# lazear/sage

Hardware: AMD Instinct MI355X
Metric: spectra/sec (whole node), fragment-index search-and-score, human tryptic narrow search (higher is better)
Workload: dtype f32

## Files before the change

include/sage_hip.h:

```cpp
#ifndef SAGE_HIP_H
#define SAGE_HIP_H

#include <stddef.h>
#include <stdint.h>

#ifdef __cplusplus
extern "C" {
#endif

#define SAGE_HIP_ABI_VERSION 6

enum {
    SAGE_HIP_OK = 0,
    SAGE_HIP_ERR_INVALID = 1,
    SAGE_HIP_ERR_NO_DEVICE = 2,
    SAGE_HIP_ERR_HIP = 3,
    SAGE_HIP_ERR_UNSUPPORTED = 4,
    SAGE_HIP_ERR_OOM = 5,
    SAGE_HIP_ERR_INTERNAL = 6
};

enum { SAGE_TOL_PPM = 0, SAGE_TOL_PCT = 1, SAGE_TOL_DA = 2 };
typedef struct SageTolerance {
    int32_t kind;
// ... 173 lines not shown

typedef struct SageTiming {
    float prelim_ms;
    float rescore_ms;
    float total_ms;
    uint32_t n_launches;
    uint32_t n_wide;
    uint32_t arena_entries;
    uint32_t n_retry;
    float retry_ms;
    uint32_t n_tied;
    uint32_t n_ways;
} SageTiming;
int sage_hip_last_timing(const SageScorer* scorer, SageTiming* out);
int sage_hip_scorer_set_timing_interval(SageScorer* scorer, uint32_t every);

int sage_hip_host_alloc(uint64_t bytes, void** out);
void sage_hip_host_free(void* p);

int sage_hip_debug_phase_cycles(SageScorer* scorer, unsigned long long* out32);
int sage_hip_debug_prune_counters(SageScorer* scorer, unsigned long long* out4);
int sage_hip_debug_filter_counters(SageScorer* scorer, unsigned long long* out4);
int sage_hip_debug_heavy_counters(SageScorer* scorer, unsigned long long* out2);

typedef struct SageRescoreInput {
    uint64_t n;
    const SageFeature* features;
    const float* aligned_rt;
    const float* delta_rt_model;
    const float* delta_ims_model;
    SageTolerance precursor_tol;
    const uint32_t* peptide_key;
    uint32_t n_peptide_keys;
    const uint32_t* protein_key;
    uint32_t n_protein_keys;
} SageRescoreInput;

typedef struct SageRescoreOutput {
    float* discriminant_score;
    float* posterior_error;
    float* spectrum_q;
    float* peptide_q;
    float* protein_q;
    uint32_t* order;
    uint64_t passing_spectrum;
    uint64_t passing_peptide;
// ... 178 lines not shown
```

sage_amd/_lib.py:

```python
import ctypes as C
import os

import numpy as np

from . import build as _build

c_float_p = C.POINTER(C.c_float)
c_u8_p = C.POINTER(C.c_uint8)
c_u32_p = C.POINTER(C.c_uint32)
c_u64_p = C.POINTER(C.c_uint64)


class SageTolerance(C.Structure):
    _fields_ = [("kind", C.c_int32), ("lo", C.c_float), ("hi", C.c_float)]


class SageTheoretical(C.Structure):
    _fields_ = [("peptide_index", C.c_uint32), ("fragment_mz", C.c_float)]


class SageDbParams(C.Structure):
    _fields_ = [
        ("bucket_size", C.c_uint64),
        ("missed_cleavages", C.c_int32),
# ... 254 lines not shown
        "sage_hip_scorer_create": (C.c_int, [vp, C.POINTER(SageScorerParams), C.POINTER(vp)]),
        "sage_hip_scorer_destroy": (None, [vp]),
        "sage_hip_scorer_clone": (C.c_int, [vp, C.POINTER(vp)]),
        "sage_hip_score_batch": (C.c_int, [vp, C.POINTER(SageSpectrumBatch), vp, c_u32_p]),
        "sage_hip_batch_upload": (C.c_int, [vp, C.POINTER(SageSpectrumBatch), C.POINTER(vp)]),
        "sage_hip_batch_free": (None, [vp]),
        "sage_hip_batch_process_upload": (C.c_int, [vp, C.POINTER(SageRawBatch), C.c_uint64, C.c_int, C.c_float, C.c_uint32,
                                                    C.POINTER(vp), c_u32_p]),
        "sage_hip_batch_download": (C.c_int, [vp, c_u64_p, c_float_p, c_float_p, c_float_p]),
        "sage_hip_batch_upload_kinds": (C.c_int, [vp, C.POINTER(SageSpectrumBatch), c_u8_p, C.POINTER(vp)]),
        "sage_hip_batch_process_upload_kinds": (C.c_int, [vp, C.POINTER(SageRawBatch), c_u8_p, C.c_uint64, C.c_int, C.c_float,
                                                          C.c_uint32, C.POINTER(vp), c_u32_p]),
        "sage_hip_score_batch_kinds": (C.c_int, [vp, C.POINTER(SageSpectrumBatch), c_u8_p, vp, c_u32_p]),
        "sage_hip_score_resident": (C.c_int, [vp, vp, vp, c_u32_p]),
        "sage_hip_initial_hits": (C.c_int, [vp, vp, c_u64_p, C.c_uint32, c_u32_p, c_u64_p, c_u64_p]),
        "sage_hip_last_timing": (C.c_int, [vp, C.POINTER(SageTiming)]),
        "sage_hip_scorer_set_timing_interval": (C.c_int, [vp, C.c_uint32]),
        "sage_hip_annotate_resident": (C.c_int, [vp, vp, vp, c_u32_p, C.POINTER(SageFragments)]),
        "sage_hip_quick_score_resident": (C.c_int, [vp, vp, C.c_int, c_u8_p]),
        "sage_hip_debug_phase_cycles": (C.c_int, [vp, c_u64_p]),
        "sage_hip_debug_prune_counters": (C.c_int, [vp, c_u64_p]),
        "sage_hip_debug_filter_counters": (C.c_int, [vp, c_u64_p]),
        "sage_hip_debug_heavy_counters": (C.c_int, [vp, c_u64_p]),
        "sage_hip_host_alloc": (C.c_int, [C.c_uint64, C.POINTER(vp)]),
        "sage_hip_host_free": (None, [vp]),
        "sage_hip_rescore": (C.c_int, [C.c_int, C.POINTER(SageRescoreInput), C.POINTER(SageRescoreOutput)]),
        "sage_hip_hostdb_competition_keys": (C.c_int, [vp, c_u32_p, C.c_uint64, c_u32_p, c_u32_p, c_u32_p, c_u32_p]),
        "sage_hip_predict_rt": (C.c_int, [C.c_int, C.POINTER(SageRtInput), C.POINTER(SageRtOutput)]),
        "sage_hip_hostdb_feature_peptides": (C.c_int, [vp, c_u32_p, C.c_uint64, c_u64_p, c_u8_p, c_float_p]),
        "sage_hip_mzml_read": (C.c_int, [C.c_char_p, C.c_uint32, C.c_int, C.POINTER(vp)]),
        "sage_hip_mzml_view": (C.c_int, [vp, C.POINTER(SageRawBatch)]),
        "sage_hip_mzml_check_searchable": (C.c_int, [vp]),
        "sage_hip_mzml_spectrum_id": (C.c_char_p, [vp, C.c_uint64]),
        "sage_hip_mzml_free": (None, [vp]),
        "sage_hip_mzml_read_sn": (C.c_int, [C.c_char_p, C.c_uint32, C.c_int, C.c_int, C.POINTER(vp)]),
        "sage_hip_mzml_ion_injection_time": (C.c_float, [vp, C.c_uint64]),
        "sage_hip_mzml_precursor_ref": (C.c_char_p, [vp, C.c_uint64]),
        "sage_hip_mgf_read": (C.c_int, [C.c_char_p, C.c_uint32, C.POINTER(vp)]),
        "sage_hip_mzml_isolation_kinds": (C.c_int, [vp, c_u8_p]),
        "sage_hip_mzml_charge_zero": (C.c_int, [vp, c_u8_p]),
        "sage_hip_parse_f32": (C.c_int, [C.c_char_p, C.c_uint64, c_float_p]),
        "sage_hip_tmt": (C.c_int, [C.c_int, C.POINTER(SageTmtInput), C.POINTER(SageTmtOutput)]),
        "sage_hip_write_tmt": (C.c_int, [C.c_char_p, C.POINTER(C.c_char_p), C.c_uint32, C.c_uint64, c_u32_p, C.POINTER(C.c_char_p),
                                         c_float_p, c_float_p, C.POINTER(C.c_char_p), C.c_uint32]),
        "sage_hip_write_results": (C.c_int, [C.c_char_p, C.c_int, vp, vp, C.c_uint64, c_u64_p, c_u64_p, C.POINTER(C.c_char_p),
                                             C.c_uint32, C.POINTER(C.c_char_p), C.POINTER(SagePostColumns)]),
# ... 3 lines not shown
        "sage_hip_mzml_has_mobility": (C.c_int, [vp, c_u8_p]),
        "sage_hip_write_lfq": (C.c_int, [C.c_char_p, vp, C.POINTER(SageLfqOutput), c_u64_p, C.c_uint64, C.POINTER(C.c_char_p),
                                         C.c_uint32]),
        "sage_hip_fasta_num_targets": (C.c_int, [C.c_char_p, C.POINTER(SageDbParams), c_u64_p]),
        "sage_hip_prefilter_chunk_size": (C.c_int, [C.c_char_p, C.POINTER(SageDbParams), C.c_uint64, c_u64_p]),
        "sage_hip_hostdb_build_chunk": (C.c_int, [C.c_char_p, C.POINTER(SageDbParams), C.c_uint64, C.c_uint64, C.POINTER(vp)]),
        "sage_hip_hostdb_merge_kept": (C.c_int, [C.POINTER(vp), C.POINTER(c_u8_p), C.c_uint32, C.POINTER(SageDbParams),
                                                 C.POINTER(vp)]),
    }
    for name, (res, args) in sig.items():
        fn = getattr(lib, name)
        fn.restype = res
        fn.argtypes = args
    _lib = lib
    return lib


EXPORTED_SYMBOLS = [
    "sage_hip_last_error", "sage_hip_abi_version", "sage_hip_hostdb_build", "sage_hip_hostdb_free",
    "sage_hip_hostdb_view", "sage_hip_hostdb_peptide_string", "sage_hip_hostdb_peptide_proteins",
    "sage_hip_hostdb_peptide_info", "sage_hip_process_ms2", "sage_hip_device_count", "sage_hip_db_create", "sage_hip_db_destroy",
    "sage_hip_db_device_bytes", "sage_hip_scorer_create", "sage_hip_scorer_destroy", "sage_hip_scorer_clone", "sage_hip_score_batch",
    "sage_hip_batch_upload", "sage_hip_batch_free", "sage_hip_batch_process_upload", "sage_hip_batch_download", "sage_hip_score_resident", "sage_hip_initial_hits",
    "sage_hip_last_timing", "sage_hip_scorer_set_timing_interval", "sage_hip_annotate_resident", "sage_hip_quick_score_resident", "sage_hip_debug_phase_cycles", "sage_hip_debug_prune_counters", "sage_hip_debug_filter_counters", "sage_hip_debug_heavy_counters", "sage_hip_host_alloc", "sage_hip_host_free",
    "sage_hip_rescore", "sage_hip_hostdb_competition_keys", "sage_hip_fasta_num_targets", "sage_hip_prefilter_chunk_size",
    "sage_hip_hostdb_build_chunk", "sage_hip_hostdb_merge_kept", "sage_hip_predict_rt", "sage_hip_hostdb_feature_peptides",
    "sage_hip_write_results", "sage_hip_mzml_read", "sage_hip_mzml_view", "sage_hip_mzml_check_searchable", "sage_hip_mzml_spectrum_id", "sage_hip_mzml_free",
    "sage_hip_lfq", "sage_hip_write_lfq", "sage_hip_mzml_read_sn", "sage_hip_mzml_ion_injection_time", "sage_hip_mzml_precursor_ref",
    "sage_hip_tmt", "sage_hip_write_tmt", "sage_hip_mgf_read", "sage_hip_mzml_isolation_kinds", "sage_hip_mzml_charge_zero",
    "sage_hip_parse_f32", "sage_hip_batch_upload_kinds", "sage_hip_batch_process_upload_kinds", "sage_hip_score_batch_kinds",
    "sage_hip_lfq_im", "sage_hip_mzml_mobility", "sage_hip_mzml_has_mobility",
]


def check(rc):
    if rc != 0:
        msg = load().sage_hip_last_error()
        raise SageHipError(f"libsage_hip status {rc}: {msg.decode() if msg else ''}")


def as_ptr(arr, ctype):
    return arr.ctypes.data_as(C.POINTER(ctype))
```

sage_amd/csrc/capi.hip:

```cpp
#include <hip/hip_runtime.h>
#include <algorithm>
#include <atomic>
#include <cmath>
#include <chrono>
#include <cstring>
#include <memory>
#include <future>
#include <mutex>
#include <string>
#include <vector>

#include "crlog.h"
#include "device_types.h"
#define HIP_FAILED(e, what) fail(status_of(e), std::string(what) + ": " + hipGetErrorString(e))
#include "hip_host.h"
#include "host_db.hpp"

using namespace sagehip;

namespace {

thread_local std::string g_last_error;

int fail(int code, const std::string& msg) {
// ... 53 lines not shown
    DevBuf<uint64_t> pm_off;
    std::vector<float> h_pep_mono;
    DevBuf<SageTheoretical> tm_frag;
    DevBuf<uint32_t> tm_lut;
    DevBuf<SageTheoretical> tm2_frag;
    DevBuf<sagecore::LutWord> tm2_l1;
    DevBuf<uint32_t> tm2_pos;
    uint32_t max_ions = 0;
    uint32_t max_len = 0;
    uint32_t ion_lo_bits = 0xFFFFFFFFu, ion_hi_bits = 0;
    DevDbView view{};
    uint64_t bytes = 0;
};

struct WorkSet {
    DevBuf<uint64_t> cand;
    DevBuf<uint32_t> cand_len, totals, status, queue, retry, item_of, ready;
    uint32_t epoch = 0;
    DevBuf<QueryRec> qrec;
    DevBuf<uint16_t> seeds;
    DevBuf<uint64_t> qres;
    DevBuf<uint32_t> arena;
    DevBuf<uint32_t> cnt_store;
    DevBuf<float> winbuf;
    DevBuf<unsigned char> hugebuf;
    uint32_t cap_tie = 0;
    uint32_t cap_n = 0;
    uint32_t cap_wide = 0;
};

struct OutSet {
    DevBuf<SageFeature> features;
    DevBuf<uint32_t> out_count;
    DevBuf<uint32_t> counters;
    uint32_t* h_counters = nullptr;
    uint32_t* h_counters_view = nullptr;
    bool counters_clean = false;
    Pinned h_out;
    Event ev[5];
    Event comp_done, down_done;
    bool in_flight = false, two_pass = false, with_rescore = false;
    bool fused = false;
    bool wide_launched = true;
    bool timed = true;
    bool retry_deferred = false;
    bool huge = false;
    uint32_t n = 0;
    ~OutSet() {
        if (h_counters) (void)hipHostFree(h_counters);
// ... 36 lines not shown
    bool retry_likely = true;
    uint32_t timing_every = 1;
    uint64_t timing_calls = 0;
    bool timed = true;
    float kept_prelim_ms = 0.f, kept_rescore_ms = 0.f, kept_retry_ms = 0.f;
    DevBuf<double> lnfact;
    DevBuf<unsigned long long> dbg;
    uint32_t tile_blocks = 0;
    uint32_t tile_blocks8 = 0;
    bool cnt8 = true;
    bool reuse_counts = true;
    SageTiming timing{};
    bool exact_always = false;
    bool one_launch = false;
    uint32_t kstride = 64;
    bool two_lanes = true;
    uint32_t search_lag = 0;
    bool sched_desc_forced = false;
    uint64_t replay_split = 0xFFFFFFFFull;
    bool fused = false;
    bool zero_copy = true;
    bool fast_ties = true;
    uint32_t cnt_stride = 0;
    uint32_t qmax = 1;
    WorkSet ws;
    WorkSet ws2;
    OutSet outs[4];
    SageDeviceBatch slots[4];
    uint32_t chunk = 131072;
    DevBuf<SageFeature> an_feats;
    DevBuf<uint32_t> an_counts;
    DevBuf<uint64_t> an_off;
    DevBuf<uint8_t> an_kinds, keep;
    DevBuf<int32_t> an_charges, an_ord;
    DevBuf<float> an_int, an_calc, an_exp;
};

extern "C" {

int sage_hip_rescore(int device, const SageRescoreInput* in, SageRescoreOutput* out) {
    if (!in || !out) return fail(SAGE_HIP_ERR_INVALID, "sage_hip_rescore: null argument");
    if (sage_hip_device_count() <= 0) return fail(SAGE_HIP_ERR_NO_DEVICE, "sage_hip_rescore: no HIP device (there is no CPU fallback)");
    if (in->n >= (1ull << 31)) return fail(SAGE_HIP_ERR_UNSUPPORTED, "sage_hip_rescore: more than 2^31 features");
    if (in->precursor_tol.kind != SAGE_TOL_PPM && in->precursor_tol.kind != SAGE_TOL_DA)
        return fail(SAGE_HIP_ERR_INVALID, "sage_hip_rescore: Pct tolerance should never be used on mz");
    out->passing_spectrum = out->passing_peptide = out->passing_protein = 0;
// ... 554 lines not shown
    s->params = *p;
    DevScorer& d = s->dev;
    d.precursor_tol = {p->precursor_tol.kind, p->precursor_tol.lo, p->precursor_tol.hi};
    d.fragment_tol = {p->fragment_tol.kind, p->fragment_tol.lo, p->fragment_tol.hi};
    d.pbm_reach = sagecore::pbm_reach_of(d.fragment_tol);
    d.min_matched_peaks = p->min_matched_peaks;
    d.min_isotope_err = p->min_isotope_err;
    d.max_isotope_err = p->max_isotope_err;
    d.min_precursor_charge = p->min_precursor_charge;
    d.max_precursor_charge = p->max_precursor_charge;
    d.override_precursor_charge = p->override_precursor_charge;
    d.max_fragment_charge = p->max_fragment_charge;
    d.chimera = p->chimera;
    d.report_psms = p->report_psms;
    d.wide_window = p->wide_window;
    d.score_type = p->score_type;
    d.kmax = std::max<uint32_t>(50, 2 * p->report_psms);
    const uint32_t n_iso = (uint32_t)(p->max_isotope_err - p->min_isotope_err) + 1;
    const uint32_t n_z = (uint32_t)(p->max_precursor_charge - p->min_precursor_charge) + 1;
    d.list_cap = d.kmax * (std::max(n_iso, n_z) + 1);
    d.wcap = 1024;
    d.dbg_flags = 0;
    if (const char* e = getenv("SAGE_HIP_DEBUG_FLAGS")) d.dbg_flags = (uint32_t)atoi(e);
    d.prune_min = (d.dbg_flags & 4096u) ? 0u : d.min_matched_peaks;
    d.rescore_general = 0;
    if (const char* e = getenv("SAGE_HIP_RESCORE_GENERAL")) d.rescore_general = atoi(e) != 0 ? 1u : 0u;
    d.exact = 0;
    d.xcd_chunk = 1024;
    if (const char* e = getenv("SAGE_HIP_XCD_CHUNK")) d.xcd_chunk = (uint32_t)std::max(0, atoi(e));
    {
        const char* e = getenv("SAGE_HIP_SCHED_DESC");
        if (!e || atoi(e)) d.xcd_chunk |= 0x80000000u;
        s->sched_desc_forced = e != nullptr;
    }
    if (const char* e = getenv("SAGE_HIP_EXACT")) s->exact_always = atoi(e) != 0;
    if (const char* e = getenv("SAGE_HIP_FUSED")) s->fused = atoi(e) != 0;
    if (const char* e = getenv("SAGE_HIP_ONE_LANE")) s->two_lanes = atoi(e) == 0;
    if (const char* e = getenv("SAGE_HIP_SEARCH_LAG")) s->search_lag = (uint32_t)std::max(0, atoi(e));
    if (const char* e = getenv("SAGE_HIP_REPLAY_WAVE_MAX")) s->replay_split = (uint64_t)atoll(e) & 0xFFFFFFFFull;
    if (const char* e = getenv("SAGE_HIP_REPLAY_LANE_MAX")) s->replay_split |= (uint64_t)(uint32_t)atoll(e) << 32;
    if (const char* e = getenv("SAGE_HIP_ONE_LAUNCH")) s->one_launch = atoi(e) != 0;
#ifndef SAGE_HIP_EXPERIMENTS
    if (s->one_launch || s->fused || getenv("SAGE_HIP_SEARCH_LAG"))
        return fail(SAGE_HIP_ERR_UNSUPPORTED, "SAGE_HIP_ONE_LAUNCH / SAGE_HIP_FUSED / SAGE_HIP_SEARCH_LAG need a build with -DSAGE_HIP_EXPERIMENTS");
#endif
    if (const char* e = getenv("SAGE_HIP_NO_ZEROCOPY")) s->zero_copy = atoi(e) == 0;
// ... 506 lines not shown
}

int sage_hip_tmt(int device, const SageTmtInput* in, SageTmtOutput* out) {
    if (!in || !out) return fail(SAGE_HIP_ERR_INVALID, "sage_hip_tmt: null argument");
    if (sage_hip_device_count() <= 0) return fail(SAGE_HIP_ERR_NO_DEVICE, "sage_hip_tmt: no HIP device (there is no CPU fallback)");
    std::string err;
    const int rc = tmt_on_device(device, *in, *out, err);
    return rc == SAGE_HIP_OK ? rc : fail(rc, err);
}

void sage_hip_batch_free(SageDeviceBatch* b) {
    if (!b) return;
    (void)hipSetDevice(b->device);
    delete b;
}

static uint64_t arena_entries_for(const SageScorer* s, uint32_t n) {
    uint64_t e = std::max<uint64_t>((uint64_t)n * 16384, 16ull << 20) + (uint64_t)std::min(n, std::max(s->tile_blocks, s->tile_blocks8)) * (2u << 16);
    e = std::min<uint64_t>(e, 0xFFFFFFF0ull);
    if (const char* v = getenv("SAGE_HIP_ARENA_MB")) e = std::min<uint64_t>((uint64_t)std::max(1, atoi(v)) << 18, 0xFFFFFFF0ull);
    return e;
}

static int ensure_work(SageScorer* s, uint32_t n, int lane, bool wide, hipStream_t st) {
    WorkSet& w = lane ? s->ws2 : s->ws;
    if (n > w.cap_n) {
        HIP_TRY(w.cand.reserve((size_t)n * s->dev.kmax + 64));
        HIP_TRY(w.cand_len.reserve(n));
        HIP_TRY(w.totals.reserve((size_t)n * 2));
        HIP_TRY(w.status.reserve(n));
        HIP_TRY(w.queue.reserve(n));
        HIP_TRY(w.retry.reserve(n));
        HIP_TRY(w.item_of.reserve(n));
        HIP_TRY(w.ready.reserve(n));
        HIP_TRY(hipMemsetAsync(w.ready.p, 0, (size_t)w.ready.n * 4, st));
        HIP_TRY(hipStreamSynchronize(st));
        w.epoch = 0;
        w.cap_n = n;
    }
    if (s->fast_ties && n > w.cap_tie) {
        const hipError_t e = w.cnt_store.reserve((size_t)n * s->cnt_stride);
        if (e == hipErrorOutOfMemory) {
            (void)hipGetLastError();
            s->fast_ties = false;
        } else {
            HIP_TRY(e);
            w.cap_tie = n;
        }
    }
    if (wide && lane == 0 && n > w.cap_wide) {
        HIP_TRY(w.qrec.reserve((size_t)n * s->qmax));
        HIP_TRY(w.seeds.reserve((size_t)n * s->qmax * s->kstride));
        HIP_TRY(w.qres.reserve((size_t)n * s->qmax * s->kstride));
        const uint64_t arena_entries = arena_entries_for(s, n);
        if (arena_entries > w.arena.n) HIP_TRY(w.arena.alloc(arena_entries));
        w.cap_wide = n;
    }
    return SAGE_HIP_OK;
}
static int ensure_out(SageScorer* s, OutSet& o, uint32_t n, bool need_features) {
    HIP_TRY(o.out_count.reserve(n));
    if (need_features) HIP_TRY(o.features.reserve((size_t)n * s->params.report_psms));
    return SAGE_HIP_OK;
}

static DevWork make_work(SageScorer* s, OutSet& o, int pass, int lane = 0) {
    DevWork w{};
    WorkSet& ws = lane ? s->ws2 : s->ws;
    w.cand = ws.cand.p;
    w.cand_len = ws.cand_len.p;
// ... 88 lines not shown
            HIP_TRY(wset.winbuf.reserve(need));
        }
    }
    o.two_pass = production && !(fused && !wide);
    o.with_rescore = with_rescore;
    o.fused = fused || one_launch;
    o.wide_launched = wide;
    o.n = view.n;
    DevBatchView v2 = view;
    v2.sched = nullptr;
    v2.sched_win = 0;
    v2.order = wset.retry.p + list_off;
    v2.n_dev = o.counters.p + CTR_RETRY;
    if (one_launch && ++wset.epoch == 0) wset.epoch = 1;
    DevWork w1 = make_work(s, o, 0, lane), w2 = make_work(s, o, 1, lane);
    for (DevWork* w : {&w1, &w2}) {
        w->queue += list_off;
        w->retry += list_off;
    }
    const bool fast_ties = s->fast_ties && production && !fused && !one_launch && o.two_pass;
    if (fast_ties) {
        w1.cnt_store = wset.cnt_store.p + (size_t)list_off * s->cnt_stride;
    }
    if (wing) w1.winbuf = w2.winbuf = wset.winbuf.p;
    o.huge = huge;
    if (huge) {
        w1.hugebuf = w2.hugebuf = wset.hugebuf.p;
        w1.huge_stride = w2.huge_stride = (uint32_t)huge_stride_bytes(sc);
    }
    if (production && s->cnt8 && !wing) {
        w1.cnt8 = 1;
        w1.tile_blocks = s->tile_blocks8;
    }
    if (production && s->reuse_counts) {
        w2.reuse = 1;
        w2.arena_ptr = w1.arena_ptr;
    }
    const SideStream side{s->side_stream, s->side_fork.e, s->side_join.e};
    DevScorer sc1 = sc, sc2 = sc;
    sc1.exact = mode == MODE_EXACT ? 1u : 0u;
    sc1.fast_log = o.two_pass ? 1u : 0u;
    sc2.exact = 1u;
    sc2.fast_log = 0u;
    const bool no_timing = !s->timed;
    o.timed = s->timed;
    o.retry_deferred = phase == 1 && o.two_pass;
// ... 595 lines not shown
}
int sage_hip_debug_filter_counters(SageScorer* s, unsigned long long* out4) {
    if (!s || !out4) return fail(SAGE_HIP_ERR_INVALID, "null argument");
    if (!s->dbg.p) return fail(SAGE_HIP_ERR_INVALID, "set SAGE_HIP_PHASE_CLOCKS=1 before creating the scorer");
    std::vector<unsigned long long> all((size_t)DBG_BLOCKS * DBG_PRUNE_WORDS);
    HIP_TRY(hipMemcpy(all.data(), s->dbg.p + (size_t)DBG_BLOCKS * 32, all.size() * 8, hipMemcpyDeviceToHost));
    for (uint32_t k = 0; k < 4; k++) out4[k] = 0;
    for (size_t b = 0; b < DBG_BLOCKS; b++)
        for (uint32_t k = 0; k < 4; k++) out4[k] += all[b * DBG_PRUNE_WORDS + 4 + k];
    return SAGE_HIP_OK;
}

int sage_hip_debug_heavy_counters(SageScorer* s, unsigned long long* out2) {
    if (!s || !out2) return fail(SAGE_HIP_ERR_INVALID, "null argument");
    if (!s->dbg.p) return fail(SAGE_HIP_ERR_INVALID, "set SAGE_HIP_PHASE_CLOCKS=1 before creating the scorer");
    std::vector<unsigned long long> all((size_t)DBG_BLOCKS * DBG_PRUNE_WORDS);
    HIP_TRY(hipMemcpy(all.data(), s->dbg.p + (size_t)DBG_BLOCKS * 32, all.size() * 8, hipMemcpyDeviceToHost));
    out2[0] = out2[1] = 0;
    for (size_t b = 0; b < DBG_BLOCKS; b++)
        for (uint32_t k = 0; k < 2; k++) out2[k] += all[b * DBG_PRUNE_WORDS + 8 + k];
    return SAGE_HIP_OK;
}

int sage_hip_host_alloc(uint64_t bytes, void** out) {
    if (!out) return fail(SAGE_HIP_ERR_INVALID, "null argument");
    HIP_TRY(hipHostMalloc(out, bytes ? bytes : 1, hipHostMallocDefault));
    if (void* d = device_view(*out)) {
        std::lock_guard<std::mutex> lock(g_blocks_mu);
        g_blocks.push_back(HostBlock{(const unsigned char*)*out, (unsigned char*)d, (size_t)(bytes ? bytes : 1)});
    }
    return SAGE_HIP_OK;
}
void sage_hip_host_free(void* p) {
    if (!p) return;
    {
        std::lock_guard<std::mutex> lock(g_blocks_mu);
        for (size_t i = 0; i < g_blocks.size(); i++)
            if (g_blocks[i].host == (const unsigned char*)p) {
                g_blocks.erase(g_blocks.begin() + (long)i);
                break;
            }
    }
    (void)hipHostFree(p);
}

int sage_hip_scorer_set_timing_interval(SageScorer* s, uint32_t every) {
// ... 35 lines not shown
```

sage_amd/csrc/device_types.h:

```cpp
#pragma once
#include <stdint.h>

#include <string>

#include "../../include/sage_hip.h"
#include "core.h"

namespace sagehip {

struct DevDbView {
    const float* pep_mono;
    uint32_t np;
    const uint32_t* pep_lut;
    uint32_t pep_lut_bins;
    float pep_lut_inv_w;
    const SageTheoretical* pm_frag;
    const uint64_t* pm_off;
    const float* ions;
    const uint64_t* ion_off;
    const uint32_t* pep_info;
    const SageTheoretical* tm_frag;
    const uint32_t* tm_lut;
    uint32_t tile_shift;
    uint32_t n_tiles;
// ... 89 lines not shown
    uint32_t cnt8;
    uint32_t reuse;
    uint32_t queue_later;
    uint32_t* item_of;
    uint32_t* ready;
    uint32_t epoch;
    uint64_t replay_split;
    uint32_t kstride;
    uint32_t search_lag;
    uint32_t* cnt_store;
    uint32_t cnt_stride;
    uint32_t* arena_ptr;
    struct QueryRec* qrec;
    uint16_t* seeds;
    uint64_t* qres;
    unsigned char* hugebuf;
    uint32_t huge_stride;
    float* winbuf;
    uint32_t* arena;
    uint32_t arena_cap;
    uint32_t qmax;
    uint32_t tile_shift;
    unsigned long long* dbg;
};

enum { ST_OK = 0, ST_DEFERRED = 1, ST_OVERFLOW = 2, ST_RETRY = 3,
       ST_DONE = 4,
       ST_OK_ORDERED = 5 };
enum { CTR_QUEUED = 0, CTR_LIST_OVERFLOW = 1, CTR_QUEUE_HEAD = 2, CTR_ARENA_PTR = 3, CTR_ARENA_OVERFLOW = 4, CTR_RETRY = 5,
       CTR_TIED = 6,
       CTR_FAST_TIE = 7,
       CTR_TIE_STRIPE0 = 16, CTR_TIE_STRIPES = 16, CTR_TIE_STRIDE = 16,
       CTR_COUNT = CTR_TIE_STRIPE0 + CTR_TIE_STRIPES * CTR_TIE_STRIDE };

struct QueryRec {
    uint32_t left;
    uint32_t potential;
    uint32_t matched;
    uint32_t scored;
    uint32_t head;
    uint32_t z_iso;
    uint32_t pad[2];
    uint32_t n_dir;
    uint32_t t0;
    uint32_t n_cand;
};

// ... 87 lines not shown
```

sage_amd/csrc/kernels.hip:

```cpp
#include <hip/hip_runtime.h>

#include <type_traits>

#include "crlog.h"
#include "device_types.h"

using namespace sagecore;

namespace sagehip {

namespace {

#ifndef SAGE_PRELIM_WAVES
#define SAGE_PRELIM_WAVES 5
#endif
#ifndef SAGE_RESCORE_WAVES
#define SAGE_RESCORE_WAVES 5
#endif
#ifndef SAGE_NARROW_WAVES
#define SAGE_NARROW_WAVES 5
#endif
#ifndef SAGE_PROBE_PER_LANE
#define SAGE_PROBE_PER_LANE 2
#endif
// ... 1117 lines not shown
    }
    for (uint32_t blk = blockIdx.x; blk < n_batch; blk += gridDim.x) {
        const uint32_t pos = xcd_position(blk, n_batch, sc.xcd_chunk);
        uint32_t spec = b.sched ? 0u : b.order ? uni(b.order[pos]) : pos;
        __syncthreads();
        Clock pc;
        pc.start((sc.dbg_flags & 512u) && !sc.exact ? nullptr : w.dbg, blk, 0);
        const SpecInfo si = b.sched ? load_spec_sched(sc, b, pos, spec) : load_spec(sc, b, spec);
        const PrelimResult r = prelim_spectrum<PROBE, BIGK, PrelimKernargs>(db, sc, b, L, si, sc.exact != 0, pc);
        typedef const __attribute__((address_space(4))) PrelimKernargs* Segment;
        Segment ka = (Segment)__builtin_amdgcn_kernarg_segment_ptr();
        asm volatile("" : "+s"(ka));
        uint32_t* const w_cnt_store = ka->w.cnt_store;
        if (!BIGK && w_cnt_store) {
            const bool keep = !r.deferred && si.z0 == si.z1 && ka->sc.min_isotope_err == ka->sc.max_isotope_err;
            uint32_t* __restrict__ row = w_cnt_store + (size_t)pos * ka->w.cnt_stride;
            if (keep && SAGE_CNT_MODE != 1)
                for (uint32_t i = lane; i < (r.q_potential + 1) / 2; i += WAVE) row[CNT_ROW_HEADER + i] = L.cnt[i];
            if (lane == 0 && SAGE_CNT_MODE != 2) {
                row[0] = keep ? r.q_left : 0u;
                row[1] = keep ? r.q_potential : 0u;
            }
        }
        if (r.deferred) {
            if (lane == 0) {
                ka->w.status[spec] = ST_DEFERRED;
                if (!ka->w.queue_later) {
                    const uint32_t it = atomicAdd(ka->w.n_deferred + CTR_QUEUED, 1u);
                    ka->w.queue[it] = spec;
                    if (!ka->w.reuse) ka->w.item_of[spec] = it;
                }
            }
            continue;
        }
        if (lane == 0) {
            if (!r.ok) atomicAdd(ka->w.n_deferred + CTR_LIST_OVERFLOW, 1u);
            ka->w.status[spec] = r.ok ? (r.untrimmed ? ST_OK_ORDERED : ST_OK) : ST_OVERFLOW;
            ka->w.cand_len[spec] = r.stored;
            ka->w.totals[2 * spec] = r.matched;
            ka->w.totals[2 * spec + 1] = r.scored;
        }
        {
            uint64_t* __restrict__ dst = ka->w.cand + (size_t)spec * ka->sc.kmax;
            for (uint32_t i = lane; i < r.stored; i += WAVE) dst[i] = L.listB[i];
        }
        pc.mark(4);
    }
}

__global__ __launch_bounds__(256) void queue_kernel(DevScorer sc, DevBatchView b, DevWork w) {
    uint32_t n_batch = b.n;
    if (b.n_dev) {
        const uint32_t nd = *b.n_dev;
        n_batch = nd < n_batch ? nd : n_batch;
    }
    const uint32_t lane = lane_id();
    for (uint32_t base = blockIdx.x * blockDim.x; base < n_batch; base += gridDim.x * blockDim.x) {
        const uint32_t blk = base + threadIdx.x;
        uint32_t spec = 0;
        bool marked = false;
        if (blk < n_batch) {
            const uint32_t pos = blk;
            spec = b.order ? b.order[pos] : pos;
            marked = w.status[spec] == ST_DEFERRED;
        }
// ... 1760 lines not shown
        asm volatile("" : "+s"(ka));
    }
    __device__ __forceinline__ const float* ions() const { return ka->db.ions; }
    __device__ __forceinline__ uint32_t report_psms() const { return ka->sc.report_psms; }
    __device__ __forceinline__ uint32_t chimera() const { return ka->sc.chimera; }
    __device__ __forceinline__ uint32_t min_matched_peaks() const { return ka->sc.min_matched_peaks; }
    __device__ __forceinline__ uint32_t prune_min() const { return ka->sc.prune_min; }
    __device__ __forceinline__ int score_type() const { return ka->sc.score_type; }
    __device__ __forceinline__ uint32_t xcd_chunk() const { return ka->sc.xcd_chunk; }
    __device__ __forceinline__ uint32_t batch_n() const { return ka->b.n; }
    __device__ __forceinline__ uint32_t spec_base() const { return ka->b.spec_base; }
    __device__ __forceinline__ uint32_t* status() const { return ka->w.status; }
    __device__ __forceinline__ uint32_t* retry() const { return ka->w.retry; }
    __device__ __forceinline__ uint32_t* counters() const { return ka->w.n_deferred; }
    __device__ __forceinline__ const uint32_t* cnt_store() const { return ka->w.cnt_store; }
    __device__ __forceinline__ uint32_t cnt_stride() const { return ka->w.cnt_stride; }
    __device__ __forceinline__ const double* lnfact_table() const { return ka->lnfact_table; }
    __device__ __forceinline__ uint32_t lnfact_n() const { return ka->lnfact_n; }
    __device__ __forceinline__ SageFeature* out() const { return ka->out; }
    __device__ __forceinline__ uint32_t* out_count() const { return ka->out_count; }
    __device__ __forceinline__ uint8_t* keep(uint8_t*) const { return ka->keep; }
};

template <bool ACC, class KA, bool FAST = false, bool CHIMERA = true, class PC>
__device__ __forceinline__ bool rescore_spectrum(const DevDbView& db, const DevScorer& sc, const DevBatchView& b, const DevWork& w,
                                                 const double* __restrict__ lnfact_table, uint32_t lnfact_n,
                                                 SageFeature* __restrict__ out, uint32_t* __restrict__ out_count,
                                                 uint8_t* __restrict__ keep, const RescoreLds& R, const uint32_t spec, uint32_t P,
                                                 const uint64_t mine, const uint32_t tot_matched, const uint32_t tot_scored,
                                                 const bool list_is_exact, const bool queue_on_tie, PC& pc) {
    const uint32_t lane = lane_id();
    uint32_t* const pbm = R.pbm;
    uint32_t* const plut = R.plut;
    float* const pm = R.pm;
    float* const pi = R.pi;
    const uint32_t pep = prescore_peptide(mine);
    const bool valid = pep != 0xFFFFFFFFu;
    const uint32_t z = prescore_charge(mine);
    const int iso = prescore_iso(mine);
    const uint32_t nfz = max_fragment_charge(sc.max_fragment_charge, z) - 1;
    uint64_t ion_base = 0;
    uint32_t lm1 = 0;
    uint32_t pep_rec = 0;
    float pep_mass = 0.0f;
    if (valid) {
        ion_base = db.ion_off[pep];
        pep_rec = db.pep_info[pep];
        pep_mass = db.pep_mono[pep];
    }
    if (lane == 0) {
        float ims = 0.0f;
        if (b.ims) { const float v = b.ims[spec]; ims = v == v ? v : 0.0f; }
        static_assert(HDR_TIC == 0 && HDR_MZP == 1 && HDR_RT == 2 && HDR_IMS == 3 && HDR_FILE == 4 && HDR_MATCHED == 5 && HDR_SCORED == 6, "two 16-byte stores");
        *(uint4*)R.hdr = make_uint4(__float_as_uint(b.tic[spec]), __float_as_uint(b.precursor_mz[spec] - PROTON) ,
                                    __float_as_uint(b.rt ? b.rt[spec] : 0.0f), __float_as_uint(ims));
        *(uint4*)(R.hdr + 4) = make_uint4(b.file_id ? b.file_id[spec] : 0u, tot_matched, tot_scored, 0u);
    }
#define SAGE_N_ITEMS (valid ? db.n_kinds * lm1 * nfz : 0u)

    double ln_lambda = 0.0;
    lds_sync();
    pc.mark(0);
    const bool sym_tol = (sc.tol_mode & TOL_SYM) != 0u;
    uint32_t nterm_mask = 0;
    for (uint32_t k = 0; k < db.n_kinds; k++) nterm_mask |= (db.ion_kinds[k] <= 2 ? 1u : 0u) << k;
    uint32_t n_emitted = 0;
    const bool any_fz2 = __ballot(valid && nfz >= 2) != 0ull, any_fz3 = __ballot(valid && nfz >= 3) != 0ull;
    for (uint32_t round = 0;; round++) {
        float inv_w;
        build_peak_lut(plut, inv_w, pm, P);
        if (round == 0 && valid) {
            const uint32_t plen = pep_rec & 0xFFFFu;
// ... 420 lines not shown
}

template <bool PROF, bool ACC, bool FAST = false, bool CHIMERA = true>
__global__ __launch_bounds__(64) SAGE_RESCORE_WAVES_ATTR void rescore_kernel(RescoreKernargs A) {
    const DevDbView& db = A.db;
    const DevScorer& sc = A.sc;
    const DevBatchView& b = A.b;
    const DevWork& w = A.w;
    const double* __restrict__ lnfact_table = A.lnfact_table;
    const uint32_t lnfact_n = A.lnfact_n;
    SageFeature* __restrict__ out = A.out;
    uint32_t* __restrict__ out_count = A.out_count;
    uint8_t* __restrict__ keep = ACC ? A.keep : nullptr;
    typedef typename std::conditional<PROF, PhaseClock, NoClock>::type Clock;
    extern __shared__ __align__(16) unsigned char smem[];
    const uint32_t lane = lane_id();
    if (blockIdx.x >= b.n) return;
    uint32_t n_batch = b.n;
    if (b.n_dev) {
        n_batch = *b.n_dev < n_batch ? *b.n_dev : n_batch;
        if (blockIdx.x >= n_batch) return;
    }
    const uint32_t pos = xcd_position(blockIdx.x, n_batch, sc.xcd_chunk);
    uint4 rec = make_uint4(0u, 0u, 0u, 0u);
    if (b.sched) rec = b.sched[(size_t)b.sched_stride * pos];
    const uint32_t spec = b.sched ? uni(rec.x) : b.order ? b.order[pos] : pos;
    const uint32_t st = w.status[spec];
    const uint64_t row_word = w.cand[(size_t)spec * sc.kmax + lane];
    const uint32_t ncand = w.cand_len[spec];
    const uint32_t tot_m = w.totals[2 * spec], tot_s = w.totals[2 * spec + 1];
    const uint64_t p0 = b.sched ? ((uint64_t)uni(rec.w) << 32) | uni(rec.z) : b.peak_off[spec];
    const uint32_t P = b.sched ? uni(rec.y) : (uint32_t)(b.peak_off[spec + 1] - p0);
    float em0 = 0.f, em1 = 0.f, em2 = 0.f, ei0 = 0.f, ei1 = 0.f, ei2 = 0.f;
    const bool early = b.sched != nullptr;
    if (early) {
        const float* __restrict__ gm = b.masses + p0;
        const float* __restrict__ gi = b.intensities + p0;
        if (lane < P) { em0 = gm[lane]; ei0 = gi[lane]; }
        if (lane + WAVE < P) { em1 = gm[lane + WAVE]; ei1 = gi[lane + WAVE]; }
        if (lane + 2 * WAVE < P) { em2 = gm[lane + 2 * WAVE]; ei2 = gi[lane + 2 * WAVE]; }
    }
    if (st == ST_DONE) return;
    if (st != ST_OK && st != ST_OK_ORDERED) {
        if (lane == 0 && !keep) out_count[spec] = 0;
        return;
    }
    const RescoreLds R = carve_rescore(smem, smem + ((rescore_scratch_bytes(keep != nullptr) + 15) & ~(size_t)15), b);
    Clock pc;
    pc.start((sc.dbg_flags & 512u) && !sc.exact ? nullptr : w.dbg, blockIdx.x, 1);
    if (early) {
        if (lane < P) { R.pm[lane] = em0; R.pi[lane] = ei0; }
        if (lane + WAVE < P) { R.pm[lane + WAVE] = em1; R.pi[lane + WAVE] = ei1; }
        if (lane + 2 * WAVE < P) { R.pm[lane + 2 * WAVE] = em2; R.pi[lane + 2 * WAVE] = ei2; }
    }
    for (uint32_t i = early ? lane + 3 * WAVE : lane; i < P; i += WAVE) {
        R.pm[i] = b.masses[p0 + i];
        R.pi[i] = b.intensities[p0 + i];
    }
    const uint64_t mine = lane < ncand ? row_word : PRESCORE_EMPTY;
    rescore_spectrum<ACC, RescoreKernargs, FAST, CHIMERA>(db, sc, b, w, lnfact_table, lnfact_n, out, out_count, keep, R, spec, P, mine, tot_m,
                                                          tot_s, sc.exact != 0 || st == ST_OK_ORDERED, true, pc);
}

#ifdef SAGE_HIP_EXPERIMENTS
constexpr uint32_t SEARCH_LAG = 8192;
struct SearchRole {
    bool rescoring;
    uint32_t v;
};
__host__ __device__ inline uint32_t search_slots(uint32_t n) { return (n + 7u) & ~7u; }
__host__ __device__ inline uint32_t search_lag(uint32_t n, uint32_t want) {
    want = want ? (want + 7u) & ~7u : SEARCH_LAG;
    return search_slots(n) < want ? search_slots(n) : want;
}
__host__ __device__ inline SearchRole search_role(uint32_t b, uint32_t n, uint32_t want_lag) {
    const uint32_t np = search_slots(n), lag = search_lag(n, want_lag);
    SearchRole r;
    if (b < lag) {
        r.rescoring = false;
        r.v = b;
    } else if (b < 2 * np - lag) {
        const uint32_t q = (b - lag) >> 3, i = (b - lag) & 7u;
        r.rescoring = (q & 1u) != 0;
// ... 46 lines not shown
        return;
    }
    const RescoreLds R = carve_rescore(smem, smem + ((rescore_scratch_bytes(false) + 15) & ~(size_t)15), b);
    Clock pc;
    pc.start(w.dbg, role.v, 1);
    const uint64_t p0 = b.peak_off[spec];
    const uint32_t P = (uint32_t)(b.peak_off[spec + 1] - p0);
    for (uint32_t i = lane; i < P; i += WAVE) {
        R.pm[i] = b.masses[p0 + i];
        R.pi[i] = b.intensities[p0 + i];
    }
    while (__hip_atomic_load(w.ready + spec, __ATOMIC_RELAXED, __HIP_MEMORY_SCOPE_AGENT) != w.epoch) __builtin_amdgcn_s_sleep(32);
    asm volatile("" ::: "memory");
    const uint32_t st = __hip_atomic_load(w.status + spec, __ATOMIC_RELAXED, __HIP_MEMORY_SCOPE_AGENT);
    if (st != ST_OK && st != ST_OK_ORDERED) {
        if (lane == 0 && st == ST_OVERFLOW) out_count[spec] = 0;
        return;
    }
    const uint32_t ncand = __hip_atomic_load(w.cand_len + spec, __ATOMIC_RELAXED, __HIP_MEMORY_SCOPE_AGENT);
    const uint32_t tot_m = __hip_atomic_load(w.totals + 2 * spec, __ATOMIC_RELAXED, __HIP_MEMORY_SCOPE_AGENT);
    const uint32_t tot_s = __hip_atomic_load(w.totals + 2 * spec + 1, __ATOMIC_RELAXED, __HIP_MEMORY_SCOPE_AGENT);
    const uint64_t mine = lane < ncand ? __hip_atomic_load(w.cand + (size_t)spec * sc.kmax + lane, __ATOMIC_RELAXED, __HIP_MEMORY_SCOPE_AGENT)
                                       : PRESCORE_EMPTY;
    const bool done = rescore_spectrum<true, void>(db, sc, b, w, lnfact_table, lnfact_n, out, out_count, nullptr, R, spec, P, mine, tot_m, tot_s,
                                       st == ST_OK_ORDERED, true, pc);
    if (done && lane == 0) w.status[spec] = ST_DONE;
}

#endif

template <bool PROBE, bool PROF>
__global__ __launch_bounds__(64) SAGE_NARROW_WAVES_ATTR void narrow_kernel(RescoreKernargs A) {
    static_assert(offsetof(RescoreKernargs, db) == offsetof(PrelimKernargs, db) && offsetof(RescoreKernargs, sc) == offsetof(PrelimKernargs, sc) &&
                      offsetof(RescoreKernargs, b) == offsetof(PrelimKernargs, b) && offsetof(RescoreKernargs, w) == offsetof(PrelimKernargs, w),
                  "the preliminary phase reads the segment as a PrelimKernargs");
    const DevDbView& db = A.db;
    const DevScorer& sc = A.sc;
    const DevBatchView& b = A.b;
    const DevWork& w = A.w;
    const double* __restrict__ lnfact_table = A.lnfact_table;
    const uint32_t lnfact_n = A.lnfact_n;
    SageFeature* __restrict__ out = A.out;
    uint32_t* __restrict__ out_count = A.out_count;
    typedef typename std::conditional<PROF, PhaseClock, NoClock>::type Clock;
    extern __shared__ __align__(16) unsigned char smem[];
    const uint32_t lane = lane_id();
    uint32_t n_batch = b.n;
// ... 21 lines not shown
            }
            const PrelimResult r = prelim_spectrum<PROBE, false, PrelimKernargs>(db, sc, b, L, si, exact, pc);
            if (r.deferred) {
                if (lane == 0) {
                    const uint32_t it = atomicAdd(w.n_deferred + CTR_QUEUED, 1u);
                    w.queue[it] = spec;
                    if (!w.reuse) w.item_of[spec] = it;
                }
                final_status = ST_DEFERRED;
                break;
            }
            if (!r.ok) {
                if (lane == 0) {
                    atomicAdd(w.n_deferred + CTR_LIST_OVERFLOW, 1u);
                    out_count[spec] = 0;
                }
                final_status = ST_OVERFLOW;
                break;
            }
            const uint64_t mine = lane < r.stored ? L.listB[lane] : PRESCORE_EMPTY;
            pc.mark(4);
            pc.rebase(1);
            __syncthreads();
            if (rescore_spectrum<true, RescoreKernargs>(db, sc, b, w, lnfact_table, lnfact_n, out, out_count, nullptr, R, spec, si.P, mine, r.matched,
                                                        r.scored, exact || r.untrimmed, false, pc) ||
                exact)
                break;
            exact = true;
            if (lane == 0) atomicAdd(w.n_deferred + CTR_TIED, 1u);
        }
        if (lane == 0) w.status[spec] = final_status;
    }
}

__global__ __launch_bounds__(256) void epilogue_kernel(const uint32_t* __restrict__ counts, uint32_t n, uint32_t* __restrict__ h_counts,
                                                       const uint32_t* __restrict__ order, EpilogueParts parts) {
    for (uint32_t i = blockIdx.x * blockDim.x + threadIdx.x; i < n; i += gridDim.x * blockDim.x) {
        const uint32_t spec = order ? order[i] : i;
        h_counts[spec] = counts[spec];
    }
    if (blockIdx.x == 0)
        for (uint32_t p = 0; p < parts.n; p++)
            for (uint32_t i = threadIdx.x; i < 2 * CTR_COUNT; i += blockDim.x) {
                parts.dst[p][i] = parts.src[p][i];
                parts.src[p][i] = 0u;
            }
}

// ... 330 lines not shown
```

Measured before the change: 152.8 million.

## Hand candidate lists to rescore via position-indexed 64-word rows

The preliminary kernel now writes each spectrum's candidate list, status, and totals into a single 64-word row indexed by schedule position, so every lane writes one word. The rescore kernel reads that row with one coalesced load, taking the header fields via lane broadcast, instead of several scattered per-spectrum loads from status, cand, cand_len and totals. Peptide metadata loads (ion offset, info, mass) are hoisted into a gather that can start before the peak loads, letting their latency overlap. It adds a workspace buffer sized per spectrum, is restricted to lists of at most 62 candidates and to the non-fused path, and has a debug flag to disable it.

```diff
diff --git a/include/sage_hip.h b/include/sage_hip.h
--- a/include/sage_hip.h
+++ b/include/sage_hip.h
@@ -219,6 +219,7 @@
 int sage_hip_debug_prune_counters(SageScorer* scorer, unsigned long long* out4);
 int sage_hip_debug_filter_counters(SageScorer* scorer, unsigned long long* out4);
 int sage_hip_debug_heavy_counters(SageScorer* scorer, unsigned long long* out2);
+int sage_hip_debug_handover_route(SageScorer* scorer, uint32_t* out);
 
 typedef struct SageRescoreInput {
     uint64_t n;
diff --git a/sage_amd/_lib.py b/sage_amd/_lib.py
--- a/sage_amd/_lib.py
+++ b/sage_amd/_lib.py
@@ -300,6 +300,7 @@
         "sage_hip_debug_prune_counters": (C.c_int, [vp, c_u64_p]),
         "sage_hip_debug_filter_counters": (C.c_int, [vp, c_u64_p]),
         "sage_hip_debug_heavy_counters": (C.c_int, [vp, c_u64_p]),
+        "sage_hip_debug_handover_route": (C.c_int, [vp, c_u32_p]),
         "sage_hip_host_alloc": (C.c_int, [C.c_uint64, C.POINTER(vp)]),
         "sage_hip_host_free": (None, [vp]),
         "sage_hip_rescore": (C.c_int, [C.c_int, C.POINTER(SageRescoreInput), C.POINTER(SageRescoreOutput)]),
@@ -349,7 +350,7 @@
     "sage_hip_hostdb_peptide_info", "sage_hip_process_ms2", "sage_hip_device_count", "sage_hip_db_create", "sage_hip_db_destroy",
     "sage_hip_db_device_bytes", "sage_hip_scorer_create", "sage_hip_scorer_destroy", "sage_hip_scorer_clone", "sage_hip_score_batch",
     "sage_hip_batch_upload", "sage_hip_batch_free", "sage_hip_batch_process_upload", "sage_hip_batch_download", "sage_hip_score_resident", "sage_hip_initial_hits",
-    "sage_hip_last_timing", "sage_hip_scorer_set_timing_interval", "sage_hip_annotate_resident", "sage_hip_quick_score_resident", "sage_hip_debug_phase_cycles", "sage_hip_debug_prune_counters", "sage_hip_debug_filter_counters", "sage_hip_debug_heavy_counters", "sage_hip_host_alloc", "sage_hip_host_free",
+    "sage_hip_last_timing", "sage_hip_scorer_set_timing_interval", "sage_hip_annotate_resident", "sage_hip_quick_score_resident", "sage_hip_debug_phase_cycles", "sage_hip_debug_prune_counters", "sage_hip_debug_filter_counters", "sage_hip_debug_heavy_counters", "sage_hip_debug_handover_route", "sage_hip_host_alloc", "sage_hip_host_free",
     "sage_hip_rescore", "sage_hip_hostdb_competition_keys", "sage_hip_fasta_num_targets", "sage_hip_prefilter_chunk_size",
     "sage_hip_hostdb_build_chunk", "sage_hip_hostdb_merge_kept", "sage_hip_predict_rt", "sage_hip_hostdb_feature_peptides",
     "sage_hip_write_results", "sage_hip_mzml_read", "sage_hip_mzml_view", "sage_hip_mzml_check_searchable", "sage_hip_mzml_spectrum_id", "sage_hip_mzml_free",
diff --git a/sage_amd/csrc/capi.hip b/sage_amd/csrc/capi.hip
--- a/sage_amd/csrc/capi.hip
+++ b/sage_amd/csrc/capi.hip
@@ -99,9 +99,11 @@
     DevBuf<uint64_t> qres;
     DevBuf<uint32_t> arena;
     DevBuf<uint32_t> cnt_store;
+    DevBuf<uint64_t> hand;
     DevBuf<float> winbuf;
     DevBuf<unsigned char> hugebuf;
     uint32_t cap_tie = 0;
+    uint32_t cap_hand = 0;
     uint32_t cap_n = 0;
     uint32_t cap_wide = 0;
 };
@@ -184,6 +186,8 @@
     bool zero_copy = true;
     bool fast_ties = true;
     uint32_t cnt_stride = 0;
+    bool hand_rows = true;
+    bool last_hand = false;
     uint32_t qmax = 1;
     WorkSet ws;
     WorkSet ws2;
@@ -784,6 +788,7 @@
     d.wcap = 1024;
     d.dbg_flags = 0;
     if (const char* e = getenv("SAGE_HIP_DEBUG_FLAGS")) d.dbg_flags = (uint32_t)atoi(e);
+    s->hand_rows = (d.dbg_flags & 131072u) == 0u;
     d.prune_min = (d.dbg_flags & 4096u) ? 0u : d.min_matched_peaks;
     d.rescore_general = 0;
     if (const char* e = getenv("SAGE_HIP_RESCORE_GENERAL")) d.rescore_general = atoi(e) != 0 ? 1u : 0u;
@@ -1336,6 +1341,10 @@
     return e;
 }
 
+static bool hand_rows_possible(const SageScorer* s) {
+    return s->hand_rows && s->dev.kmax <= HAND_LIST_MAX && !s->dev.big_path && !s->fused && !s->one_launch && !s->exact_always;
+}
+
 static int ensure_work(SageScorer* s, uint32_t n, int lane, bool wide, hipStream_t st) {
     WorkSet& w = lane ? s->ws2 : s->ws;
     if (n > w.cap_n) {
@@ -1360,6 +1369,18 @@
         } else {
             HIP_TRY(e);
             w.cap_tie = n;
+        }
+    }
+    if (!wide && hand_rows_possible(s) && n > w.cap_hand) {
+        const hipError_t e = w.hand.reserve((size_t)n * HAND_ROW_WORDS);
+        if (e == hipErrorOutOfMemory) {
+            (void)hipGetLastError();
+            s->hand_rows = false;
+        } else {
+            HIP_TRY(e);
+            HIP_TRY(hipMemsetAsync(w.hand.p, 0, w.hand.bytes(), st));
+            HIP_TRY(hipStreamSynchronize(st));
+            w.cap_hand = n;
         }
     }
     if (wide && lane == 0 && n > w.cap_wide) {
@@ -1494,6 +1515,10 @@
     if (fast_ties) {
         w1.cnt_store = wset.cnt_store.p + (size_t)list_off * s->cnt_stride;
     }
+    const bool hand_on = production && !fused && !one_launch && !wide && !huge && view.sched != nullptr && hand_rows_possible(s) &&
+                         (uint64_t)list_off + view.n <= wset.cap_hand;
+    if (hand_on) w1.hand = wset.hand.p + (size_t)list_off * HAND_ROW_WORDS;
+    if (phase != 2) s->last_hand = hand_on;
     if (wing) w1.winbuf = w2.winbuf = wset.winbuf.p;
     o.huge = huge;
     if (huge) {
@@ -2135,6 +2160,12 @@
     return SAGE_HIP_OK;
 }
 
+int sage_hip_debug_handover_route(SageScorer* s, uint32_t* out) {
+    if (!s || !out) return fail(SAGE_HIP_ERR_INVALID, "null argument");
+    *out = s->last_hand ? 1u : 0u;
+    return SAGE_HIP_OK;
+}
+
 int sage_hip_host_alloc(uint64_t bytes, void** out) {
     if (!out) return fail(SAGE_HIP_ERR_INVALID, "null argument");
     HIP_TRY(hipHostMalloc(out, bytes ? bytes : 1, hipHostMallocDefault));
diff --git a/sage_amd/csrc/device_types.h b/sage_amd/csrc/device_types.h
--- a/sage_amd/csrc/device_types.h
+++ b/sage_amd/csrc/device_types.h
@@ -135,7 +135,12 @@
     uint32_t qmax;
     uint32_t tile_shift;
     unsigned long long* dbg;
-};
+    uint64_t* hand;
+};
+constexpr uint32_t HAND_ROW_WORDS = 64, HAND_HEAD_WORD = 62, HAND_TOTALS_WORD = 63, HAND_LIST_MAX = HAND_HEAD_WORD;
+static_assert(HAND_LIST_MAX <= HAND_HEAD_WORD && HAND_HEAD_WORD < HAND_TOTALS_WORD && HAND_TOTALS_WORD < HAND_ROW_WORDS && HAND_ROW_WORDS == 64,
+              "the list and the two header words fit a row of one word per lane");
+static_assert(HAND_ROW_WORDS * sizeof(uint64_t) % 128 == 0, "rows keep the array's 128-byte alignment");
 
 enum { ST_OK = 0, ST_DEFERRED = 1, ST_OVERFLOW = 2, ST_RETRY = 3,
        ST_DONE = 4,
diff --git a/sage_amd/csrc/kernels.hip b/sage_amd/csrc/kernels.hip
--- a/sage_amd/csrc/kernels.hip
+++ b/sage_amd/csrc/kernels.hip
@@ -1163,6 +1163,15 @@
                 row[1] = keep ? r.q_potential : 0u;
             }
         }
+        uint64_t* const w_hand = BIGK ? nullptr : ka->w.hand;
+        if (w_hand) {
+            const uint32_t st = r.deferred ? (uint32_t)ST_DEFERRED : r.ok ? (r.untrimmed ? (uint32_t)ST_OK_ORDERED : (uint32_t)ST_OK) : (uint32_t)ST_OVERFLOW;
+            const uint32_t stored = r.deferred ? 0u : (r.stored < HAND_LIST_MAX ? r.stored : HAND_LIST_MAX);
+            uint64_t v = lane < stored ? L.listB[lane] : PRESCORE_EMPTY;
+            if (lane == HAND_HEAD_WORD) v = (uint64_t)stored << 32 | st;
+            if (lane == HAND_TOTALS_WORD) v = r.deferred ? 0ull : (uint64_t)r.scored << 32 | r.matched;
+            w_hand[(size_t)pos * HAND_ROW_WORDS + lane] = v;
+        }
         if (r.deferred) {
             if (lane == 0) {
                 ka->w.status[spec] = ST_DEFERRED;
@@ -1174,14 +1183,14 @@
             }
             continue;
         }
-        if (lane == 0) {
-            if (!r.ok) atomicAdd(ka->w.n_deferred + CTR_LIST_OVERFLOW, 1u);
-            ka->w.status[spec] = r.ok ? (r.untrimmed ? ST_OK_ORDERED : ST_OK) : ST_OVERFLOW;
-            ka->w.cand_len[spec] = r.stored;
-            ka->w.totals[2 * spec] = r.matched;
-            ka->w.totals[2 * spec + 1] = r.scored;
-        }
-        {
+        if (lane == 0 && !r.ok) atomicAdd(ka->w.n_deferred + CTR_LIST_OVERFLOW, 1u);
+        if (!w_hand) {
+            if (lane == 0) {
+                ka->w.status[spec] = r.ok ? (r.untrimmed ? ST_OK_ORDERED : ST_OK) : ST_OVERFLOW;
+                ka->w.cand_len[spec] = r.stored;
+                ka->w.totals[2 * spec] = r.matched;
+                ka->w.totals[2 * spec + 1] = r.scored;
+            }
             uint64_t* __restrict__ dst = ka->w.cand + (size_t)spec * ka->sc.kmax;
             for (uint32_t i = lane; i < r.stored; i += WAVE) dst[i] = L.listB[i];
         }
@@ -2988,12 +2997,28 @@
     __device__ __forceinline__ uint8_t* keep(uint8_t*) const { return ka->keep; }
 };
 
+struct CandGather {
+    uint64_t ion_base;
+    uint32_t pep_rec;
+    float pep_mass;
+};
+__device__ __forceinline__ CandGather gather_candidate(const DevDbView& db, const uint64_t mine) {
+    CandGather g{0ull, 0u, 0.0f};
+    const uint32_t pep = prescore_peptide(mine);
+    if (pep != 0xFFFFFFFFu) {
+        g.ion_base = db.ion_off[pep];
+        g.pep_rec = db.pep_info[pep];
+        g.pep_mass = db.pep_mono[pep];
+    }
+    return g;
+}
+
 template <bool ACC, class KA, bool FAST = false, bool CHIMERA = true, class PC>
 __device__ __forceinline__ bool rescore_spectrum(const DevDbView& db, const DevScorer& sc, const DevBatchView& b, const DevWork& w,
                                                  const double* __restrict__ lnfact_table, uint32_t lnfact_n,
                                                  SageFeature* __restrict__ out, uint32_t* __restrict__ out_count,
                                                  uint8_t* __restrict__ keep, const RescoreLds& R, const uint32_t spec, uint32_t P,
-                                                 const uint64_t mine, const uint32_t tot_matched, const uint32_t tot_scored,
+                                                 const uint64_t mine, const CandGather& cg, const uint32_t tot_matched, const uint32_t tot_scored,
                                                  const bool list_is_exact, const bool queue_on_tie, PC& pc) {
     const uint32_t lane = lane_id();
     uint32_t* const pbm = R.pbm;
@@ -3005,15 +3030,10 @@
     const uint32_t z = prescore_charge(mine);
     const int iso = prescore_iso(mine);
     const uint32_t nfz = max_fragment_charge(sc.max_fragment_charge, z) - 1;
-    uint64_t ion_base = 0;
     uint32_t lm1 = 0;
-    uint32_t pep_rec = 0;
-    float pep_mass = 0.0f;
-    if (valid) {
-        ion_base = db.ion_off[pep];
-        pep_rec = db.pep_info[pep];
-        pep_mass = db.pep_mono[pep];
-    }
+    const uint64_t ion_base = cg.ion_base;
+    const uint32_t pep_rec = cg.pep_rec;
+    const float pep_mass = cg.pep_mass;
     if (lane == 0) {
         float ims = 0.0f;
         if (b.ims) { const float v = b.ims[spec]; ims = v == v ? v : 0.0f; }
@@ -3480,13 +3500,31 @@
         if (blockIdx.x >= n_batch) return;
     }
     const uint32_t pos = xcd_position(blockIdx.x, n_batch, sc.xcd_chunk);
+    const uint64_t* __restrict__ const hand = w.hand;
+    uint64_t row_word = 0;
+    if (hand) row_word = hand[(size_t)pos * HAND_ROW_WORDS + lane];
     uint4 rec = make_uint4(0u, 0u, 0u, 0u);
     if (b.sched) rec = b.sched[(size_t)b.sched_stride * pos];
+    uint32_t st, ncand, tot_m, tot_s;
+    uint64_t mine = PRESCORE_EMPTY;
+    CandGather cg{0ull, 0u, 0.0f};
+    if (hand) {
+        const uint64_t head = lane_value(row_word, HAND_HEAD_WORD), totals = lane_value(row_word, HAND_TOTALS_WORD);
+        st = (uint32_t)head;
+        ncand = (uint32_t)(head >> 32);
+        tot_m = (uint32_t)totals;
+        tot_s = (uint32_t)(totals >> 32);
+        mine = lane < ncand && lane < HAND_LIST_MAX ? row_word : PRESCORE_EMPTY;
+        cg = gather_candidate(db, mine);
+    }
     const uint32_t spec = b.sched ? uni(rec.x) : b.order ? b.order[pos] : pos;
-    const uint32_t st = w.status[spec];
-    const uint64_t row_word = w.cand[(size_t)spec * sc.kmax + lane];
-    const uint32_t ncand = w.cand_len[spec];
-    const uint32_t tot_m = w.totals[2 * spec], tot_s = w.totals[2 * spec + 1];
+    if (!hand) {
+        st = w.status[spec];
+        row_word = w.cand[(size_t)spec * sc.kmax + lane];
+        ncand = w.cand_len[spec];
+        tot_m = w.totals[2 * spec];
+        tot_s = w.totals[2 * spec + 1];
+    }
     const uint64_t p0 = b.sched ? ((uint64_t)uni(rec.w) << 32) | uni(rec.z) : b.peak_off[spec];
     const uint32_t P = b.sched ? uni(rec.y) : (uint32_t)(b.peak_off[spec + 1] - p0);
     float em0 = 0.f, em1 = 0.f, em2 = 0.f, ei0 = 0.f, ei1 = 0.f, ei2 = 0.f;
@@ -3515,8 +3553,11 @@
         R.pm[i] = b.masses[p0 + i];
         R.pi[i] = b.intensities[p0 + i];
     }
-    const uint64_t mine = lane < ncand ? row_word : PRESCORE_EMPTY;
-    rescore_spectrum<ACC, RescoreKernargs, FAST, CHIMERA>(db, sc, b, w, lnfact_table, lnfact_n, out, out_count, keep, R, spec, P, mine, tot_m,
+    if (!hand) {
+        mine = lane < ncand ? row_word : PRESCORE_EMPTY;
+        cg = gather_candidate(db, mine);
+    }
+    rescore_spectrum<ACC, RescoreKernargs, FAST, CHIMERA>(db, sc, b, w, lnfact_table, lnfact_n, out, out_count, keep, R, spec, P, mine, cg, tot_m,
                                                           tot_s, sc.exact != 0 || st == ST_OK_ORDERED, true, pc);
 }
 
@@ -3609,7 +3650,8 @@
     const uint32_t tot_s = __hip_atomic_load(w.totals + 2 * spec + 1, __ATOMIC_RELAXED, __HIP_MEMORY_SCOPE_AGENT);
     const uint64_t mine = lane < ncand ? __hip_atomic_load(w.cand + (size_t)spec * sc.kmax + lane, __ATOMIC_RELAXED, __HIP_MEMORY_SCOPE_AGENT)
                                        : PRESCORE_EMPTY;
-    const bool done = rescore_spectrum<true, void>(db, sc, b, w, lnfact_table, lnfact_n, out, out_count, nullptr, R, spec, P, mine, tot_m, tot_s,
+    const bool done = rescore_spectrum<true, void>(db, sc, b, w, lnfact_table, lnfact_n, out, out_count, nullptr, R, spec, P, mine,
+                                                   gather_candidate(db, mine), tot_m, tot_s,
                                        st == ST_OK_ORDERED, true, pc);
     if (done && lane == 0) w.status[spec] = ST_DONE;
 }
@@ -3677,8 +3719,8 @@
             pc.mark(4);
             pc.rebase(1);
             __syncthreads();
-            if (rescore_spectrum<true, RescoreKernargs>(db, sc, b, w, lnfact_table, lnfact_n, out, out_count, nullptr, R, spec, si.P, mine, r.matched,
-                                                        r.scored, exact || r.untrimmed, false, pc) ||
+            if (rescore_spectrum<true, RescoreKernargs>(db, sc, b, w, lnfact_table, lnfact_n, out, out_count, nullptr, R, spec, si.P, mine,
+                                                        gather_candidate(db, mine), r.matched, r.scored, exact || r.untrimmed, false, pc) ||
                 exact)
                 break;
             exact = true;
```

Result: faster. 155.1 million, median of 6 (+1.5%).
